# amidos2006/gym-pcgrl

Measured on AMD Instinct MI355X. Metric: env-steps/sec (whole node), binary-narrow 14x14 @ 65536 envs, higher is better.
Workload: dtype u8; 1 GPU; binary-narrow-v0 14x14, 65536 envs/GPU; envs_per_gpu=65536, width=14, height=14, max_changes=39, actions=uniform random, device-generated before the timed region, parallelism=env-axis shard x1, no collective on the step path

## Files before the change

gym_pcgrl_amd/_lib.py:

```python
import ctypes as C
import os
import subprocess

PKG = os.path.dirname(os.path.abspath(__file__))
ROOT = os.path.dirname(PKG)
CSRC = os.path.join(PKG, "csrc")
LIBDIR = os.path.join(PKG, "lib")
SO = os.path.join(LIBDIR, "libpcgrl_hip.so")
SOURCES = [os.path.join(CSRC, "pcgrl_abi.hip")]
HIPCC_FLAGS = ["--offload-arch=gfx950", "-O3", "-std=c++17", "-ffp-contract=off", "-fPIC", "-shared", "-mllvm", "-amdgpu-sched-strategy=max-ilp"]

PCGRL_OK, PCGRL_EINVAL, PCGRL_EHIP, PCGRL_ESTATE = 0, -1, -2, -3


class Config(C.Structure):
    _fields_ = [(n, C.c_int32) for n in (
        "prob", "rep", "num_envs", "width", "height", "prob_width", "prob_height", "max_changes", "max_iterations",
        "random_start", "random_tile", "warp", "random_probs", "auto_reset", "target_path",
        "max_enemies", "target_enemy_dist", "max_crates", "target_solution", "solver_power", "max_potions",
        "max_treasures", "max_diamonds", "min_spikes", "target_jumps", "min_empty", "min_enemies", "min_jumps")] + [
        ("target_col_enemies", C.c_double), ("tile_probs", C.c_double * 8), ("rewards", C.c_double * 12)]


class Layout(C.Structure):
    _fields_ = [(n, C.c_int32) for n in ("group", "mask_bytes", "nplanes", "nstats")] + [
        (n, C.c_size_t) for n in ("map", "old_map", "heatmap", "pos", "planes", "counters", "stats", "start_stats",
                                  "info", "reward", "done", "tile_p", "rng_rep", "rng_prob", "rng_cursor", "scratch")]


TUNING_FIELDS = ("no_fused", "fused_zelda", "step_epb", "no_inc", "inline_reset", "pair_min", "no_wide", "wide_waves", "wide_grid",
                 "wide_pairs", "wide_few", "sok_generic", "sok_hard_cap", "sok_spawn", "md_only_agent", "smb_lds_heap", "full_per_wave", "inc_per_wave", "wide_spin", "step_prio", "no_touch", "touch_tight", "step_pair", "async_split", "big_team", "obs_at_end")


class Tuning(C.Structure):
    _fields_ = [(n, C.c_int32) for n in TUNING_FIELDS]


TUNING_OVERRIDES = {}


def make_tuning(overrides=None):
    t = Tuning(*([-1] * len(TUNING_FIELDS)))
    for k, v in list(TUNING_OVERRIDES.items()) + list((overrides or {}).items()):
        if k not in TUNING_FIELDS:
            raise KeyError("unknown tuning switch %r (known: %s)" % (k, ", ".join(TUNING_FIELDS)))
        setattr(t, k, int(v))
    return t


BUFFER_NAMES = ("map", "old_map", "heatmap", "pos", "planes", "counters", "stats", "start_stats", "info", "reward",
                "done", "tile_p", "rng_rep", "rng_prob", "rng_cursor", "scratch")


class Buffers(C.Structure):
    _fields_ = [(n, C.c_void_p) for n in BUFFER_NAMES]


ROW_FIELDS = ("actions_out", "reward", "done", "start_in", "start_out", "ep_return", "ep_length", "took", "fresh")


class Row(C.Structure):
    _fields_ = [(n, C.c_void_p) for n in ROW_FIELDS] + [("actions_i64", C.c_int32)]


class RenderDesc(C.Structure):
    _fields_ = [("indices", C.c_void_p), ("count", C.c_int32), ("tiles", C.c_void_p), ("tile_size", C.c_int32),
                ("border_x", C.c_int32), ("border_y", C.c_int32), ("border_tile", C.c_int32), ("cursor", C.c_int32),
                ("grid_rows", C.c_int32), ("grid_cols", C.c_int32), ("out", C.c_void_p)]


ABI_VERSION = 15
EXPORTS = ("pcgrl_abi_version", "pcgrl_error_string", "pcgrl_last_hip_error", "pcgrl_query_layout", "pcgrl_create",
           "pcgrl_destroy", "pcgrl_bind", "pcgrl_configure", "pcgrl_seed", "pcgrl_set_tile_probs", "pcgrl_reset",
           "pcgrl_step", "pcgrl_set_maps", "pcgrl_observe", "pcgrl_action_map", "pcgrl_status", "pcgrl_profile",
           "pcgrl_profile_read", "pcgrl_bind_episode_stats", "pcgrl_seed_words", "pcgrl_rollout", "pcgrl_bind_observation", "pcgrl_selftest_heap",
           "pcgrl_tuning_defaults", "pcgrl_set_tuning", "pcgrl_clear_status", "pcgrl_step_flat",
           "pcgrl_async_bytes", "pcgrl_bind_async", "pcgrl_step_async", "pcgrl_async_flush", "pcgrl_step_multi", "pcgrl_selftest_step_pool", "pcgrl_step_threads", "pcgrl_selftest_range_reward",
           "pcgrl_bind_row", "pcgrl_render", "pcgrl_get_stats_bytes", "pcgrl_get_stats", "pcgrl_get_reward",
           "pcgrl_get_solution_bytes", "pcgrl_get_solution")
NPHASE = 6
PHASES = ("update", "stats", "reset_or_idle", "solver_or_reset", "reset2", "solver2")


def sources_newer_than_lib():
# ... 130 lines not shown
```

gym_pcgrl_amd/csrc/kernels_stats.h:

```cpp
#pragma once
template <class MaskT>
__device__ __forceinline__ MaskT row_valid(int lane, int W, int H) {
    MaskT full = (W >= (int)(8 * sizeof(MaskT))) ? ~(MaskT)0 : (((MaskT)1 << W) - 1);
    return lane < H ? full : (MaskT)0;
}

template <int PROB = -1>
__device__ __forceinline__ bool finalize_item(const PcgrlParams& P, const DevBufs& B, int e, const int32_t* s,
                                              int mode, int parity, int shard, bool push_reset = true, int rst_list = WL_RST,
                                              const int2* pre = nullptr, const double* reward_pre = nullptr) {
    const int prob = PROB >= 0 ? PROB : P.prob;
    int32_t* st = B.stats + (size_t)e * 8;
    int32_t* start = B.start_stats + (size_t)e * 8;
    if (mode == MODE_STEP) {
        int32_t old[PCGRL_MAX_STATS], sv[PCGRL_MAX_STATS];
        for (int k = 0; k < 8; k++) { old[k] = st[k]; sv[k] = start[k]; }
        const int2 c = pre ? *pre : reinterpret_cast<const int2*>(B.counters)[e];
        const double r = reward_pre ? *reward_pre : compute_reward(P, s, old, prob);
        const bool d = episode_over(P, s, sv, prob) || c.y >= P.max_changes || c.x >= P.max_iterations;
        B.reward[e] = r;
        B.done[e] = d ? 1 : 0;
        episode_account(B, e, r, d);
        int32_t* inf = B.info + (size_t)e * 10;
#pragma unroll
// ... 118 lines not shown
            MaskT t0, t1, t2;
            reset_rows_to_planes<MaskT>(P, reinterpret_cast<MaskT*>(B.planes) + (size_t)ek * NPL * G, gw == 2 * k + 1 ? g.lane : -1, rr.m0, rr.m1, rr.m2, t0, t1, t2);
            if (gw == 2 * k + 1) { b0 = t0; b1 = t1; b2 = t2; }
            __builtin_amdgcn_wave_barrier();
        }
        TL(9);
        const bool act = have && (role == 1 || !reset_only);
        int32_t sl[PCGRL_MAX_STATS] = {0, 0, 0, 0, 0, 0, 0, 0};
        MaskT champ_l = 0;
        bool ns = false;
        if (act) ns = compute_item_stats<PROB>(g, P, b0, b1, b2, rowmask, sl, champ_l, (B.step_tight & 2) != 0);
        TL(10);
        constexpr bool kLaneReward = PROB == PCGRL_PROB_ZELDA && G == 16;
        double rpre = 0.0;
        if (kLaneReward && SL && role == 0 && act) rpre = zelda_reward_lanes(&SL->zr, B.stats + (size_t)e * 8, sl, g.lane);
        if (g.lane == 0 && role == 0 && act) finalize_item<PROB>(P, B, e, sl, MODE_STEP, parity, shard, false, WL_RST, &pre, (kLaneReward && SL) ? &rpre : nullptr);
        __builtin_amdgcn_wave_barrier();
        if (role == 1 && have) {
            if (kInc && champ_base) champ_base[(size_t)e * G + g.lane] = champ_l;
            if (g.lane == 0) finish_or_park<PROB>(P, B, e, sl, ns, MODE_START, parity, shard);
        }
        if (FUSED && step_obs) {
#pragma unroll
            for (int k = 0; k < GPW / 2; k++) {
                if (k > 0 && !pair) break;
                if (!__builtin_amdgcn_readlane((int)have, 2 * k * G)) continue;
                const ObsPlanes<MaskT, NPL> src = {reinterpret_cast<const MaskT*>(B.planes), G};
                obs_write_env_lean(src, obs_view_from_lds(&SL->obs_v), B.pos, __builtin_amdgcn_readlane(e, 2 * k * G), lane64);
            }
        }
        return;
    }
    int32_t s[PCGRL_MAX_STATS] = {0, 0, 0, 0, 0, 0, 0, 0};
    bool need_solver = false;
    MaskT champ = 0;
    if (kInc && inc) {
        if (compute) {
            const MaskT cbit = (g.lane == wl_inc_row<G>(raw)) ? (MaskT)1 << wl_inc_col<G>(raw) : (MaskT)0;
            const MaskT champ_old = champ_base[(size_t)e * G + g.lane];
            const int4 old = *reinterpret_cast<const int4*>(B.stats + (size_t)e * 8);
            int regions, path, ub2;
            binary_incremental(g, (MaskT)(~b0 & rowmask), cbit, wl_inc_code<G>(raw) != 0, old.x, old.y, champ_old, old.w - 1, regions, path, champ, ub2);
            s[0] = regions; s[1] = path; s[2] = 1; s[3] = ub2 + 1;
        }
    } else if (kZinc && packed) {
        if (compute) {
            const MaskT cbit = (g.lane == wl_inc_row<G>(raw)) ? (MaskT)1 << wl_inc_col<G>(raw) : (MaskT)0;
            zelda_stats(g, P, b0, b1, b2, rowmask, s, (int)wl_inc_code<G>(raw), cbit, B.stats[(size_t)e * 8 + 4]);
        }
    } else {
        bool full = compute;
        if (kInc && G == 16) {
            const bool t = compute && tch;
            if (t) {
                const MaskT cbit = (g.lane == wl_inc_row<G>(raw)) ? (MaskT)1 << wl_inc_col<G>(raw) : (MaskT)0;
                const MaskT champ_old = champ_base[(size_t)e * G + g.lane];
                const int4 old = *reinterpret_cast<const int4*>(B.stats + (size_t)e * 8);
                int regions, path, ub2;
                if (binary_touch(g, (MaskT)(~b0 & rowmask), cbit, (wl_inc_code<G>(raw) & 1u) != 0, old.x, champ_old, old.w - 1, regions, path, champ, ub2)) {
                    s[0] = regions; s[1] = path; s[2] = 1; s[3] = ub2 + 1;
                    full = false;
                }
            }
        }
        if (full) need_solver = compute_item_stats<PROB>(g, P, b0, b1, b2, rowmask, s, champ, (B.step_tight & 1) != 0);
    }
    if (kInc && compute && champ_base) champ_base[(size_t)e * G + g.lane] = champ;
    TL(10);
    int want_reset = 0;
    constexpr bool kLaneReward = PROB == PCGRL_PROB_ZELDA && G == 16;
    double rpre = 0.0;
    const bool lane_reward = kLaneReward && SL != nullptr && mode == MODE_STEP;
    if (lane_reward && have && !reset_only) rpre = zelda_reward_lanes(&SL->zr, B.stats + (size_t)e * 8, s, g.lane);
    if (g.lane == 0 && have) {
        if (reset_only) want_reset = 1;
        else want_reset = finish_or_park<PROB>(P, B, e, s, need_solver, mode, parity, shard, !inline_reset, -1, lane_reward ? &rpre : nullptr) ? 1 : 0;
    }
    if (inline_reset) {
        const uint64_t want = __ballot(want_reset != 0);
        TL(11);
        if (want) {
            TL(12);
            if (SL) { while (__hip_atomic_load(&SL->refill_done[SL->par], __ATOMIC_ACQUIRE, __HIP_MEMORY_SCOPE_WORKGROUP) < SL->need) __builtin_amdgcn_s_sleep(2); }
            bool mine = false;
#pragma unroll
            for (int k = 0; k < GPW; k++) {
                if ((want >> (k * G)) & 1ull) {
                    const int ek = __builtin_amdgcn_readlane(e, k * G);
                    if (SL && lane64 == 0) { SL->dirty[ek - SL->e0] = 1; SL->late[ek - SL->e0] = 1; SL->n_late = 1; }
                    int pend = 0;
                    if (SL) {
                        if (lane64 == 0) {
                            pend = atomicExch(&SL->pend[ek - SL->e0], 0);
                            if (pend < 0) {
                                while (__hip_atomic_load(&SL->late_done[(ek - SL->e0) >> 6], __ATOMIC_ACQUIRE, __HIP_MEMORY_SCOPE_WORKGROUP) == 0) __builtin_amdgcn_s_sleep(2);
                                pend = 0;
                            }
                        }
                        pend = __builtin_amdgcn_readfirstlane(pend);
                    }
                    ResetRows rr;
                    wave_reset_env<PROB, !FUSED, FUSED>(P, B, ek, gen_map, mt, (uint8_t*)nullptr, lane64, 0, gw == k ? g.lane : -1, &rr, pend);
                    MaskT t0, t1, t2;
                    reset_rows_to_planes<MaskT>(P, reinterpret_cast<MaskT*>(B.planes) + (size_t)ek * NPL * G, gw == k ? g.lane : -1, rr.m0, rr.m1, rr.m2, t0, t1, t2);
                    if (gw == k) { b0 = t0; b1 = t1; b2 = t2; mine = true; }
                    __builtin_amdgcn_wave_barrier();
                }
            }
            if (mine) {
                int32_t st[PCGRL_MAX_STATS] = {0, 0, 0, 0, 0, 0, 0, 0};
                const bool ns = compute_item_stats<PROB>(g, P, b0, b1, b2, rowmask, st, champ, (B.step_tight & 2) != 0);
                if (kInc && champ_base) champ_base[(size_t)e * G + g.lane] = champ;
                if (g.lane == 0) finish_or_park<PROB>(P, B, e, st, ns, MODE_START, parity, shard);
            }
        }
// ... 316 lines not shown
```

gym_pcgrl_amd/csrc/pcgrl_abi.hip:

```cpp
#include <hip/hip_runtime.h>
#include <stdio.h>
#include <stdlib.h>
#include <string.h>

#include <vector>

#include "../../include/pcgrl_hip.h"

#ifdef PCGRL_PART
#define PCGRL_IN_PART(k) (PCGRL_PART == (k))
#else
#define PCGRL_IN_PART(k) 1
#endif
#define PCGRL_LOCAL __attribute__((visibility("hidden")))
#define PART_CORE 0
#define PART_STATS 1
#define PART_UPDATE 2
#define PART_STEP_BINARY 3
#define PART_STEP_ZELDA 4
#define PART_SEARCH 5
#define PART_SMB 6
#define PART_STEP_SOLVER 7

#include "lanegroup_dev.h"
// ... 222 lines not shown
        S.sok_env = b.take(align_up((size_t)c->num_envs * (SOK_RES_WORDS + SOK_CNT_WORDS + SOK_STOP_WORDS) * 4, 256));
        S.sok_sync = b.take(align_up(2 * (size_t)(SOK_SY_WORDS + SOK_HARD_CAP) * 4, 256));
        if (!big && !sok_in_lds(c)) {
            S.sok_heap = b.take(SOK_BLOCKS * sok_heap_bytes(c->solver_power));
            S.sok_table = b.take(SOK_BLOCKS * (size_t)sok_table_size(c->solver_power) * 4);
        }
    }
    S.champ = b.take(champ_bytes(c));
    const size_t n = (size_t)c->num_envs;
    S.fifo = b.take(c->rep == PCGRL_NARROW ? align_up(n * PCGRL_FIFO_N * 4, 256) : 0);
    S.fifo_tag = b.take(c->rep == PCGRL_NARROW ? align_up(n * 4, 256) : 0);
    S.wide_sync = b.take((c->prob == PCGRL_BINARY && c->height > 16 && !big_map(c)) ? align_up(n * 16, 256) : 0);
    S.total = b.off;
    return S;
}

PCGRL_LOCAL int search_device_setup(pcgrl_env* h);
PCGRL_LOCAL int smb_device_setup(pcgrl_env* h);
#if PCGRL_IN_PART(PART_CORE)
static int device_setup(pcgrl_env* h) {
    {
        uint32_t tab[PCGRL_MT_N];
        tab[0] = 19650218u;
        for (int i = 1; i < PCGRL_MT_N; i++) tab[i] = 1812433253u * (tab[i - 1] ^ (tab[i - 1] >> 30)) + (uint32_t)i;
        HIPCHK(hipMemcpyToSymbol(HIP_SYMBOL(g_mt_genrand), tab, sizeof(tab)));
    }
    if (h->cfg.prob == PCGRL_SMB) return smb_device_setup(h);
    if (solver_prob(h->cfg.prob) && !big_search(&h->cfg)) return search_device_setup(h);
    return PCGRL_OK;
}

static void resolve_tuning(pcgrl_env* h) {
    const pcgrl_tuning& T = h->tun;
    DevBufs& B = h->B;
    h->no_wide = tun_or(T.no_wide, 0) ? 1 : 0;
    h->wide_waves = tun_or(T.wide_waves, 8);
    h->wide_pairs = tun_or(T.wide_pairs, 1);
    h->wide_grid = tun_or(T.wide_grid, 2048);
    if (h->wide_grid < 1) h->wide_grid = 2048;
    h->fused_zelda = tun_or(T.fused_zelda, 1) ? 1 : 0;
    h->no_fused = tun_or(T.no_fused, 0) ? 1 : 0;
    h->obs_at_end = tun_or(T.obs_at_end, 0) ? 1 : 0;
    h->async_split = tun_or(T.async_split, h->cfg.prob == PCGRL_SOKOBAN ? 1 : 0) ? 1 : 0;
    const int n_ = h->cfg.num_envs;
    h->step_epb = T.step_epb > 0 ? T.step_epb : ((n_ >= 192 * 256 && n_ <= 256 * 256) ? 256 : (n_ >= 192 * 128 ? 128 : 64));
    if (h->step_epb != 128 && h->step_epb != 256) h->step_epb = 64;
    h->smb_heap = T.smb_lds_heap > 0 ? T.smb_lds_heap : SMB_LDS_HEAP;
    if (h->smb_heap < 256 || h->smb_heap > 4096) h->smb_heap = SMB_LDS_HEAP;
    const int f = tun_or(T.full_per_wave, 4), i = tun_or(T.inc_per_wave, 4);
    B.step_fpw = (f == 1 || f == 2) ? f : 4;
    B.step_prio = tun_or(T.step_prio, h->cfg.prob == PCGRL_BINARY ? (h->cfg.rep == PCGRL_NARROW ? (15 | (3 << 6)) : 15) : 0) & 0xFFF;
    B.step_ipw = (i == 1 || i == 2) ? i : 4;
    B.step_touch = tun_or(T.no_touch, 0) ? 0 : 1;
    B.step_pair = tun_or(T.step_pair, 6);
    B.step_tight = B.step_touch ? tun_or(T.touch_tight, 1) : 0;
    h->no_inc = tun_or(T.no_inc, 0) != 0;
    B.zelda_inc = (h->cfg.prob == PCGRL_ZELDA && h->cfg.rep <= PCGRL_REP_TURTLE && h->cfg.height <= 16 && h->cfg.width <= 32 &&
                   h->cfg.num_envs <= WL_INC_ENV_MASK && !h->no_inc) ? 1 : 0;
    B.pair_min = tun_or(T.pair_min, 2048);
    B.big_team = tun_or(T.big_team, 1) ? 1 : 0;
    h->big_team_waves = tun_or(T.big_team, 1) >= 2 ? (tun_or(T.big_team, 1) > BIG_TEAM_MAX_WAVES ? BIG_TEAM_MAX_WAVES : tun_or(T.big_team, 1)) : 4;
    B.wide_few = tun_or(T.wide_few, WL_WIDE_FEW_REGIONS);
    B.wide_spin = T.wide_spin > 0 ? T.wide_spin : WIDE_SPIN_LIMIT;
    B.inline_reset = (!solver_prob(h->cfg.prob) && tun_or(T.inline_reset, 1) != 0) ? 1 : 0;
    if (big_search(&h->cfg)) {
        B.sok_fast_maxc = -1; B.md_only_agent = -1; B.sok_hard_cap = 0; B.sok_spawn_iters = SOK_SPAWN_ITERS;
    } else if (solver_prob(h->cfg.prob)) {
        B.sok_fast_maxc = tun_or(T.sok_generic, 0) ? -1 : SOKF_MAXC;
        B.md_only_agent = T.md_only_agent;
        B.sok_hard_cap = tun_or(T.sok_hard_cap, SOK_HARD_CAP);
        B.sok_spawn_iters = T.sok_spawn > 0 ? T.sok_spawn : SOK_SPAWN_ITERS;
        if (B.sok_hard_cap > SOK_HARD_CAP) B.sok_hard_cap = SOK_HARD_CAP;
    }
}
static int bind_buffers(pcgrl_env* h, const pcgrl_buffers* b, hipStream_t st) {
    const pcgrl_config& c = h->cfg;
    DevBufs& B = h->B;
    B.map = (uint8_t*)b->map; B.old_map = (uint8_t*)b->old_map; B.heat = (uint16_t*)b->heatmap; B.pos = (uint8_t*)b->pos;
    B.heat_end = B.heat + (size_t)c.num_envs * c.width * c.height;
    B.heat32 = c.auto_reset ? 0 : 1;
    B.ep_return = nullptr; B.ep_length = nullptr; B.last_return = nullptr; B.last_length = nullptr;
    B.planes = b->planes; B.counters = (int32_t*)b->counters; B.stats = (int32_t*)b->stats;
    B.start_stats = (int32_t*)b->start_stats; B.info = (int32_t*)b->info; B.reward = (double*)b->reward;
    B.done = (uint8_t*)b->done; B.tile_p = (double*)b->tile_p; B.rng_rep = (uint32_t*)b->rng_rep;
    B.rng_prob = (uint32_t*)b->rng_prob; B.rng_cur = (int32_t*)b->rng_cursor;
    B.obs = ObsSpec{nullptr, 0, 0, 0, 0, 0, 0, 0};
    B.local = nullptr; B.flat = nullptr;
    const ScratchPlan S = scratch_plan(&c);
    uint8_t* s = (uint8_t*)b->scratch;
    B.wl_cnt = at<int32_t>(s, S.wl_cnt); B.status = at<int32_t>(s, S.status);
    for (int k = 0; k < WL_NLIST; k++) { B.wl_cap[k] = wl_capacity(c.num_envs, k); B.wl_items[k] = at<int32_t>(s, S.wl_items[k]); }
    HIPCHK(hipMemsetAsync(B.wl_cnt, 0, S.wl_cnt.bytes + S.status.bytes, st));
    B.champ = h->no_inc ? nullptr : at<uint8_t>(s, S.champ);
    if (B.champ) HIPCHK(hipMemsetAsync(B.champ, c.prob == PCGRL_SMB ? 0xFF : 0, S.champ.bytes, st));
    B.fifo = at<uint32_t>(s, S.fifo); B.fifo_tag = at<int32_t>(s, S.fifo_tag);
    if (B.fifo_tag) HIPCHK(hipMemsetAsync(B.fifo_tag, 0xFF, S.fifo_tag.bytes, st));
    B.wide_sync = at<int32_t>(s, S.wide_sync); B.wide_epoch = 0;
    if (B.wide_sync) HIPCHK(hipMemsetAsync(B.wide_sync, 0, S.wide_sync.bytes, st));
    const bool big = big_search(&c);
    B.big_arena = big ? at<uint8_t>(s, S.arena) : nullptr;
    B.sok_pool = big ? nullptr : at<SokNode>(s, S.arena);
    B.sok_heap = at<uint32_t>(s, S.sok_heap); B.sok_table = at<uint32_t>(s, S.sok_table);
    if (solver_prob(c.prob)) {
        const int power = h->alloc_solver_power = c.solver_power;
        h->big_dims = S.big;
        B.sok_res = at<int32_t>(s, S.sok_env);
// ... 1243 lines not shown
```

gym_pcgrl_amd/csrc/pcgrl_algos.h:

```cpp
#pragma once
#include "pcgrl_common.h"

#if defined(__HIPCC__) && defined(__HIP_DEVICE_COMPILE__)
#define PCGRL_NO_IFCVT() asm volatile("" ::: "memory")
#else
#define PCGRL_NO_IFCVT() do {} while (0)
#endif
#ifndef PCGRL_TRACE
#define PCGRL_TRACE(g, site)
#endif

struct PcgrlParams {
    int32_t prob, rep, num_envs, width, height, ntiles, nplanes, group, mask_bytes;
    int32_t max_changes, max_iterations;
    int32_t random_start, random_tile, warp, random_probs, auto_reset;
    int32_t target_path, max_enemies, target_enemy_dist, max_crates, target_solution, solver_power;
    int32_t prob_width, prob_height;
    int32_t max_potions, max_treasures;
    int32_t max_diamonds, min_spikes, target_jumps;
    int32_t min_empty, min_enemies, min_jumps;
    int32_t big, big_search;
    double target_col_enemies;
    double rewards[PCGRL_MAX_REWARDS];
    double cdf[PCGRL_MAX_TILES];
// ... 374 lines not shown
template <class B>
PCGRL_D void regions_and_longest_path(B& g, typename B::mask_t pass, int& regions, int& path) {
    typename B::mask_t champ;
    regions_and_longest_path(g, pass, regions, path, champ);
}

template <class B>
PCGRL_D void binary_incremental(B& g, typename B::mask_t pass_new, typename B::mask_t cbit, bool added, int regions_old, int path_old,
                                typename B::mask_t champ_old, int ub2_old, int& regions, int& path, typename B::mask_t& champ, int& ub2) {
    typedef typename B::mask_t M;
    const M base = pass_new & ~cbit;
    M rest = pcg_neighbours(g, cbit) & base;
    path = path_old;
    champ = champ_old;
    constexpr bool kTrack = B::kGroup == 16;
    const bool track = kTrack && ub2_old >= 0;
    int k = 0, ub = track ? ub2_old : 0;
    M uni = cbit;
    if (g.any(rest)) {
        const PcgFillCtx<B> ctx = pcg_fill_ctx(g, base);
        while (g.any(rest)) {
            const M comp = pcg_component(g, g.first_bit(rest), ctx);
            rest = rest & ~comp;
            ++k;
            if (added) uni = uni | comp;
            else {
                int bd = g.popcount_sum(comp) - 1, e = 0;
                const int thr = track ? ub : path;
                if (bd > thr) e = pcg_double_sweep(g, comp, thr, bd);
                if (e > path) { if (kTrack) ub = path > ub ? path : ub; path = e; champ = comp; }
                else if (kTrack) ub = bd > ub ? bd : ub;
            }
        }
    }
    if (added) {
        regions = regions_old + 1 - k;
        int bd = g.popcount_sum(uni) - 1, e = 0;
        const int thr = track ? ub : path;
        if (bd > thr) e = pcg_double_sweep(g, uni, thr, bd);
        if (e > path) { if (kTrack) ub = path > ub ? path : ub; path = e; champ = uni; }
        else if (kTrack) ub = bd > ub ? bd : ub;
    } else {
        regions = regions_old + k - 1;
    }
    ub2 = track ? ub : -1;
}
template <class B>
PCGRL_D void binary_incremental(B& g, typename B::mask_t pass_new, typename B::mask_t cbit, bool added, int regions_old, int path_old,
                                typename B::mask_t champ_old, int& regions, int& path, typename B::mask_t& champ) {
    int ub2;
    binary_incremental(g, pass_new, cbit, added, regions_old, path_old, champ_old, -1, regions, path, champ, ub2);
}

template <class B>
PCGRL_D bool binary_touch(B& g, typename B::mask_t pass_new, typename B::mask_t cbit, bool added, int regions_old,
                          typename B::mask_t champ_old, int ub2_old, int& regions, int& path, typename B::mask_t& champ, int& ub2) {
    typedef typename B::mask_t M;
    const M base = pass_new & ~cbit;
    const M dom = added ? (base & ~champ_old) : (champ_old & ~cbit);
    M rest = pcg_neighbours(g, cbit) & dom;
    int k = 0, size1 = 0, size2 = 0, size3 = 0;
    M uni = cbit ^ cbit, big1 = uni, big2 = uni;
    if (g.any(rest)) {
        const PcgFillCtx<B> ctx = pcg_fill_ctx(g, dom);
        while (g.any(rest)) {
            const M comp = pcg_component(g, g.first_bit(rest), ctx);
            rest = rest & ~comp;
            ++k;
            uni = uni | comp;
            const int size = g.popcount_sum(comp);
            if (size > size1) { size3 = size2; size2 = size1; big2 = big1; size1 = size; big1 = comp; }
            else if (size > size2) { size3 = size2; size2 = size; big2 = comp; }
            else if (size > size3) size3 = size;
        }
    }
    const M target = added ? (champ_old | cbit | uni) : big1;
    int e = pcg_double_sweep(g, target, added ? ub2_old - 1 : -1);
    bool ok = true;
    int ub = ub2_old;
    champ = target;
    if (added) {
        regions = regions_old - k;
    } else {
        regions = regions_old + k - 1;
        ok = k > 0;
        if (size2 > 0) {
            int bd = size2 - 1, e2 = 0;
            const int thr = e < ub ? e : ub;
            if (bd > thr) e2 = pcg_double_sweep(g, big2, thr, bd);
            if (e2 > e) { ub = e > ub ? e : ub; e = e2; champ = big2; }
            else ub = bd > ub ? bd : ub;
        }
        if (size3 > 0) {
            if (size3 - 1 > e) ok = false;
            else ub = size3 - 1 > ub ? size3 - 1 : ub;
        }
    }
    path = e;
    ub2 = ub;
    return ok && e >= ub2_old;
}

template <class B>
PCGRL_D typename B::mask_t rlp_choose_seed(B& g, typename B::mask_t rest, int row_lo, int row_hi) {
    const typename B::mask_t mine = g.rows_between(rest, row_lo, row_hi);
    return g.first_bit(g.any(mine) ? mine : rest);
}
#if defined(PCGRL_TIMELINE) && defined(__HIPCC__)
__device__ __forceinline__ void tl_mark(int tag);
#define PCGRL_TLA(tag) tl_mark(tag)
#else
#define PCGRL_TLA(tag) do {} while (0)
#endif
#if defined(__HIPCC__) && defined(__HIP_DEVICE_COMPILE__) && !defined(PCGRL_EXP_NO_SWEEP_PRIO)
#define PCGRL_SWEEP_PRIO(p) __builtin_amdgcn_s_setprio(p)
#else
#define PCGRL_SWEEP_PRIO(p) do {} while (0)
#endif
template <class B, class Shared>
PCGRL_D void rlp_process_seed(B& g, typename B::mask_t seed, const PcgFillCtx<B>& ctx, Shared& sh, int& regions, int& my_best,
                              typename B::mask_t& my_champ) {
    typedef typename B::mask_t M;
    const M comp = pcg_component(g, seed, ctx);
    PCGRL_TLA(30);
    if (!sh.retire(g, comp)) return;
    ++regions;
    const int best = sh.best();
    if (g.popcount_sum(comp) - 1 > best) {
        PCGRL_TLA(31);
        PCGRL_SWEEP_PRIO(3);
        const int e = pcg_double_sweep(g, comp, best);
        PCGRL_SWEEP_PRIO(0);
        if (e > my_best) { my_best = e; my_champ = comp; }
        sh.raise(e);
        PCGRL_TLA(32);
    }
}
template <class B, class Shared>
PCGRL_D void rlp_process_seed(B& g, typename B::mask_t seed, const PcgFillCtx<B>& ctx, Shared& sh, int& regions) {
    int my_best = 0;
    typename B::mask_t my_champ = seed ^ seed;
    rlp_process_seed(g, seed, ctx, sh, regions, my_best, my_champ);
}
template <class B>
PCGRL_D typename B::mask_t rlp_prepare(B& g, typename B::mask_t pass, int& tiny_regions, int& tiny_path) {
    tiny_regions = 0; tiny_path = 0;
    return pass & ~pcg_tiny_components(g, pass, tiny_regions, tiny_path);
}

template <class M>
struct ZeldaMasks {
    M empty, solid, player, key, door, enemy;
};
// ... 137 lines not shown
```

gym_pcgrl_amd/csrc/worklist.h:

```cpp
#pragma once
#define PCGRL_BLOCK 256
#define PCGRL_STATUS_TOO_MANY_CRATES 1
#define PCGRL_STATUS_BAD_ACTION 2
#define PCGRL_STATUS_BAD_TILE 4
enum { MODE_STEP = 0, MODE_START = 1, MODE_SETMAP = 2 };

#define WL_NSHARD 64
#define WL_WIDE_FEW_REGIONS 32
#define WL_CSTRIDE 16
enum { WL_CHG = 0, WL_RST = 1, WL_SOL = 2, WL_SOL2 = 3, WL_RST2 = 4, WL_SOL3 = 5, WL_INC = 6, WL_NLIST = 7 };
#ifndef SMB_LONG_POPS
#define SMB_LONG_POPS 2000
#endif
#define WL_INC_ENV_MASK 0x1FFFFF
#define WL_INC64_ENV_MASK 0x7FFFF
__device__ __forceinline__ int wl_inc_pack(int group, int e, int row, int col, unsigned code) {
    return group == 16 ? (int)((unsigned)e | ((unsigned)(row * 32 + col) << 21) | (code << 30))
                       : (int)((unsigned)e | ((unsigned)(row * 64 + col) << 19) | ((code & 1u) << 31));
}
#define WL_INCBIG_ENV_MASK 0x7FFF
__device__ __forceinline__ int wl_incbig_pack(int e, int x, int y, bool added) { return (int)((unsigned)e | ((unsigned)x << 15) | ((unsigned)y << 23) | (added ? 0x80000000u : 0u)); }
template <int G> __device__ __forceinline__ int wl_inc_env(int raw) { return raw & (G == 16 ? WL_INC_ENV_MASK : WL_INC64_ENV_MASK); }
template <int G> __device__ __forceinline__ int wl_inc_row(int raw) { return G == 16 ? ((raw >> 26) & 15) : ((raw >> 25) & 63); }
template <int G> __device__ __forceinline__ int wl_inc_col(int raw) { return G == 16 ? ((raw >> 21) & 31) : ((raw >> 19) & 63); }
// ... 19 lines not shown
        const int i = s_tl_idx[wv];
        if (i < TL_SLOTS) { g_tl_buf[((size_t)blockIdx.x * (blockDim.x >> 6) + wv) * TL_SLOTS + i] = ((unsigned long long)wall_clock64() << 8) | (unsigned)tag; s_tl_idx[wv] = i + 1; }
    }
}
#define TL_INIT() do { if ((threadIdx.x & 63) == 0) s_tl_idx[threadIdx.x >> 6] = 0; } while (0)
#define TL(tag) tl_mark(tag)
#else
#define TL_INIT() do {} while (0)
#define TL(tag) do {} while (0)
#endif

struct LocalLists;
struct ObsSpec { uint8_t* out; int32_t oh, ow, depth, centered, pad;
                 int32_t fused,
                         delta; };
struct RowBind { int64_t* actions_out; double* reward; uint8_t* done; const uint8_t* start_in; uint8_t* start_out;
                 double* ep_return; int32_t* ep_length; uint8_t* took; uint8_t* fresh; };
struct DevBufs {
    uint8_t* map; uint8_t* old_map; uint16_t* heat; uint8_t* pos; void* planes;
    void* champ;
    int32_t* wide_sync;
    int32_t wide_spin;
    int32_t wide_few;
    int32_t wide_epoch;
    const uint16_t* heat_end;
    double* ep_return; int32_t* ep_length; double* last_return; int32_t* last_length;
    int32_t* counters; int32_t* stats; int32_t* start_stats; int32_t* info;
    double* reward; uint8_t* done; double* tile_p;
    uint32_t* rng_rep; uint32_t* rng_prob; int32_t* rng_cur;
    int32_t* wl_cnt;
    int32_t* wl_items[WL_NLIST];
    int32_t wl_cap[WL_NLIST];
    SokNode* sok_pool; uint32_t* sok_heap; uint32_t* sok_table; int32_t* status;
    int32_t* sok_res;
    int32_t* sok_cnt; int32_t* sok_stop;
    struct LocalLists* local;
    int32_t md_only_agent;
    int32_t* sok_sync;
    int32_t sok_pool_stride, sok_heap_stride, sok_table_size, sok_use_lds;
    int32_t sok_spawn_iters;
    int32_t sok_hard_cap;
    int32_t sok_fast_maxc;
    int32_t inline_reset;
    int32_t pair_min;
    int32_t zelda_inc;
    uint32_t* fifo; int32_t* fifo_tag;
    ObsSpec obs;
    int32_t step_fpw, step_ipw;
    int32_t step_prio;
    int32_t step_tight;
    const int32_t* flat;
    int32_t step_pair;
    int32_t big_team;
    int32_t step_touch;
    uint8_t* big_arena;
    uint8_t* pending; unsigned long long* async_stats;
    const uint8_t* async_slots; size_t async_slot_bytes; int32_t async_nslots; int32_t* async_run; int32_t* async_run_n;
    int32_t heat32;
    RowBind row; int32_t act_i64;
};
#define PCGRL_FIFO_N 8

struct ZeldaRewardTab { double w[8]; int lo[8]; int hi[8]; };
struct ObsView {
    uint8_t* out;
    int oh, ow, depth, centered, pad, W, H;
};
struct StepLocal {
    int e0;
    int par, need;
    int refill_done[2];
    int pend[256];
    int late_done[4];
    uint8_t dirty[256];
    uint8_t obs_skip[256];
    uint8_t late[256];
    int n_late;
    ObsView obs_v;
    ZeldaRewardTab zr;
};

__device__ __forceinline__ void async_list_runnable(const DevBufs& B, int gi) {
    if (gi < B.async_nslots && __hip_atomic_load(reinterpret_cast<const int32_t*>(B.async_slots + (size_t)gi * B.async_slot_bytes), __ATOMIC_RELAXED, __HIP_MEMORY_SCOPE_AGENT) == 1)
        B.async_run[atomicAdd(B.async_run_n, 1)] = gi;
}
__device__ __forceinline__ int32_t* wl_counters(const DevBufs& B, int parity, int list) {
    return B.wl_cnt + (size_t)(parity * WL_NLIST + list) * WL_NSHARD * WL_CSTRIDE;
}
#define WL_LOCAL_CAP 512
struct LocalLists { int n[WL_NLIST]; int e0; uint16_t items[WL_NLIST][WL_LOCAL_CAP]; };
__device__ __forceinline__ void wl_push(const DevBufs& B, int parity, int list, int shard, int value) {
    if (B.local) {
        const int i = atomicAdd(&B.local->n[list], 1);
        B.local->items[list][i] = (uint16_t)(value - B.local->e0);
        return;
    }
    const int i = atomicAdd(wl_counters(B, parity, list) + shard * WL_CSTRIDE, 1);
    B.wl_items[list][(size_t)shard * B.wl_cap[list] + i] = value;
}
__device__ __forceinline__ int wl_load_prefix(const DevBufs& B, int parity, int list, int* s_pref) {
    if (threadIdx.x < WL_NSHARD) {
        int v = wl_counters(B, parity, list)[threadIdx.x * WL_CSTRIDE];
        for (int o = 1; o < WL_NSHARD; o <<= 1) {
            const int t = __shfl_up(v, o, 64);
            if ((int)threadIdx.x >= o) v += t;
        }
// ... 163 lines not shown
```

include/pcgrl_hip.h:

```cpp
#ifndef PCGRL_HIP_H
#define PCGRL_HIP_H
#include <stddef.h>
#include <stdint.h>

#ifdef __cplusplus
extern "C" {
#endif

#define PCGRL_ABI_VERSION 15
#define PCGRL_OK 0
#define PCGRL_EINVAL (-1)
#define PCGRL_EHIP (-2)
#define PCGRL_ESTATE (-3)

enum { PCGRL_BINARY = 0, PCGRL_ZELDA = 1, PCGRL_SOKOBAN = 2, PCGRL_MDUNGEON = 3, PCGRL_DDAVE = 4, PCGRL_SMB = 5 };
enum { PCGRL_NARROW = 0, PCGRL_WIDE = 1, PCGRL_TURTLE = 2, PCGRL_NARROW_CAST = 3, PCGRL_NARROW_MULTI = 4, PCGRL_TURTLE_CAST = 5 };

typedef struct pcgrl_config {
    int32_t prob, rep;
    int32_t num_envs;
    int32_t width, height;
    int32_t prob_width, prob_height;
    int32_t max_changes, max_iterations;
    int32_t random_start, random_tile, warp, random_probs;
// ... 16 lines not shown
    int32_t nstats;
    size_t map;
    size_t old_map;
    size_t heatmap;
    size_t pos;
    size_t planes;
    size_t counters;
    size_t stats;
    size_t start_stats;
    size_t info;
    size_t reward;
    size_t done;
    size_t tile_p;
    size_t rng_rep;
    size_t rng_prob;
    size_t rng_cursor;
    size_t scratch;
} pcgrl_layout;

typedef struct pcgrl_buffers {
    void *map, *old_map, *heatmap, *pos, *planes, *counters, *stats, *start_stats, *info, *reward,
         *done, *tile_p, *rng_rep, *rng_prob, *rng_cursor, *scratch;
} pcgrl_buffers;

typedef struct pcgrl_env pcgrl_env;

typedef struct pcgrl_tuning {
    int32_t no_fused;
    int32_t fused_zelda;
    int32_t step_epb;
    int32_t no_inc;
    int32_t inline_reset;
    int32_t pair_min;
    int32_t no_wide;
    int32_t wide_waves;
    int32_t wide_grid;
    int32_t wide_pairs;
    int32_t wide_few;
    int32_t sok_generic;
    int32_t sok_hard_cap;
    int32_t sok_spawn;
    int32_t md_only_agent;
    int32_t smb_lds_heap;
    int32_t full_per_wave;
    int32_t inc_per_wave;
    int32_t wide_spin;
    int32_t step_prio;
    int32_t no_touch;
    int32_t touch_tight;
    int32_t step_pair;
    int32_t async_split;
    int32_t big_team;
    int32_t obs_at_end;
} pcgrl_tuning;

int pcgrl_abi_version(void);
const char* pcgrl_error_string(int code);
int pcgrl_last_hip_error(void);

int pcgrl_query_layout(const pcgrl_config* cfg, pcgrl_layout* out);
int pcgrl_create(const pcgrl_config* cfg, pcgrl_env** out);
int pcgrl_destroy(pcgrl_env* env);
void pcgrl_tuning_defaults(pcgrl_tuning* t);
int pcgrl_set_tuning(pcgrl_env* env, const pcgrl_tuning* t);
int pcgrl_bind(pcgrl_env* env, const pcgrl_buffers* bufs, void* stream);
int pcgrl_configure(pcgrl_env* env, const pcgrl_config* cfg);
int pcgrl_seed(pcgrl_env* env, const uint32_t* keys, int32_t first, int32_t count, void* stream);
int pcgrl_seed_words(pcgrl_env* env, const uint32_t* words, int32_t first, int32_t count, void* stream);
int pcgrl_set_tile_probs(pcgrl_env* env, void* stream);
int pcgrl_reset(pcgrl_env* env, void* stream);
int pcgrl_step(pcgrl_env* env, const int32_t* actions, void* stream);
int pcgrl_step_multi(pcgrl_env* const* envs, const int32_t* const* actions, void* const* streams, int32_t count);
int32_t pcgrl_step_threads(int32_t n);
int pcgrl_rollout(pcgrl_env* env, const int32_t* actions, int32_t steps, double* reward_out, uint8_t* done_out,
                  int32_t* info_out, void* stream);
int pcgrl_set_maps(pcgrl_env* env, const uint8_t* maps, void* stream);
int pcgrl_observe(pcgrl_env* env, uint8_t* out, int32_t out_h, int32_t out_w, int32_t centered, int32_t pad_value,
                  int32_t onehot, void* stream);
int pcgrl_bind_observation(pcgrl_env* env, uint8_t* out, int32_t out_h, int32_t out_w, int32_t centered,
                           int32_t pad_value, int32_t onehot, int32_t incremental);
typedef struct pcgrl_row {
    int64_t* actions_out;
    double*  reward;
    uint8_t* done;
    const uint8_t* start_in;
    uint8_t* start_out;
    double*  ep_return;
    int32_t* ep_length;
    uint8_t* took;
    uint8_t* fresh;
    int32_t  actions_i64;
} pcgrl_row;
int pcgrl_bind_row(pcgrl_env* env, const pcgrl_row* row);
typedef struct pcgrl_render_desc {
    const int32_t* indices;
    int32_t count;
    const uint8_t* tiles;
    int32_t tile_size;
    int32_t border_x, border_y, border_tile, cursor;
    int32_t grid_rows, grid_cols;
    uint8_t* out;
} pcgrl_render_desc;
int pcgrl_render(pcgrl_env* env, const pcgrl_render_desc* d, void* stream);
size_t pcgrl_get_stats_bytes(const pcgrl_config* cfg, int32_t count);
int    pcgrl_get_stats(pcgrl_env* env, const uint8_t* maps, int32_t count, int32_t* rows_out,
                       void* work, size_t work_bytes, void* stream);
// ... 30 lines not shown
```

Baseline: 2.309 billion env-steps/s.

## Resume longest-path search from touch-pass memo instead of full recompute

When the incremental touch update of the binary path/region stats cannot conclude, the step now resumes the region and longest-path computation from a memo of components and double-sweep results already found, instead of falling back to the full compute_item_stats pass. The resume skips re-sweeping known components and prunes remaining components by size bounds. This adds a new switch (on by default, only for the fused 32-bit mask path) and more register state carried through the touch routine, which could raise register pressure or introduce correctness risk in the bound logic.

```diff
diff --git a/gym_pcgrl_amd/_lib.py b/gym_pcgrl_amd/_lib.py
--- a/gym_pcgrl_amd/_lib.py
+++ b/gym_pcgrl_amd/_lib.py
@@ -29,7 +29,7 @@
 
 
 TUNING_FIELDS = ("no_fused", "fused_zelda", "step_epb", "no_inc", "inline_reset", "pair_min", "no_wide", "wide_waves", "wide_grid",
-                 "wide_pairs", "wide_few", "sok_generic", "sok_hard_cap", "sok_spawn", "md_only_agent", "smb_lds_heap", "full_per_wave", "inc_per_wave", "wide_spin", "step_prio", "no_touch", "touch_tight", "step_pair", "async_split", "big_team", "obs_at_end")
+                 "wide_pairs", "wide_few", "sok_generic", "sok_hard_cap", "sok_spawn", "md_only_agent", "smb_lds_heap", "full_per_wave", "inc_per_wave", "wide_spin", "step_prio", "no_touch", "touch_tight", "step_pair", "async_split", "big_team", "obs_at_end", "touch_resume")
 
 
 class Tuning(C.Structure):
diff --git a/gym_pcgrl_amd/csrc/kernels_stats.h b/gym_pcgrl_amd/csrc/kernels_stats.h
--- a/gym_pcgrl_amd/csrc/kernels_stats.h
+++ b/gym_pcgrl_amd/csrc/kernels_stats.h
@@ -194,15 +194,31 @@
         bool full = compute;
         if (kInc && G == 16) {
             const bool t = compute && tch;
+            TouchMemo<MaskT> memo = touch_memo_empty(g, b0);
             if (t) {
                 const MaskT cbit = (g.lane == wl_inc_row<G>(raw)) ? (MaskT)1 << wl_inc_col<G>(raw) : (MaskT)0;
                 const MaskT champ_old = champ_base[(size_t)e * G + g.lane];
                 const int4 old = *reinterpret_cast<const int4*>(B.stats + (size_t)e * 8);
                 int regions, path, ub2;
-                if (binary_touch(g, (MaskT)(~b0 & rowmask), cbit, (wl_inc_code<G>(raw) & 1u) != 0, old.x, champ_old, old.w - 1, regions, path, champ, ub2)) {
+                if (binary_touch(g, (MaskT)(~b0 & rowmask), cbit, (wl_inc_code<G>(raw) & 1u) != 0, old.x, champ_old, old.w - 1, regions, path, champ, ub2, memo)) {
                     s[0] = regions; s[1] = path; s[2] = 1; s[3] = ub2 + 1;
                     full = false;
                 }
+            }
+#ifdef PCGRL_TIMELINE
+            {
+                const uint64_t gu = __ballot(t && full && g.lane == 0), pl = __ballot(compute && !tch && g.lane == 0);
+                TL(32 + __popcll(gu) + 8 * __popcll(pl));
+            }
+#endif
+            constexpr bool kResume = FUSED && sizeof(MaskT) == 4;
+            if (kResume && B.touch_resume) {
+                if (full) {
+                    int regions, path, ub2;
+                    rlp_resume(g, (MaskT)(~b0 & rowmask), memo, regions, path, champ, ub2, (B.step_tight & 1) != 0);
+                    s[0] = regions; s[1] = path; s[2] = g.any(champ) ? 1 : 0; s[3] = ub2 + 1;
+                }
+                full = false;
             }
         }
         if (full) need_solver = compute_item_stats<PROB>(g, P, b0, b1, b2, rowmask, s, champ, (B.step_tight & 1) != 0);
diff --git a/gym_pcgrl_amd/csrc/pcgrl_abi.hip b/gym_pcgrl_amd/csrc/pcgrl_abi.hip
--- a/gym_pcgrl_amd/csrc/pcgrl_abi.hip
+++ b/gym_pcgrl_amd/csrc/pcgrl_abi.hip
@@ -298,6 +298,7 @@
     B.step_prio = tun_or(T.step_prio, h->cfg.prob == PCGRL_BINARY ? (h->cfg.rep == PCGRL_NARROW ? (15 | (3 << 6)) : 15) : 0) & 0xFFF;
     B.step_ipw = (i == 1 || i == 2) ? i : 4;
     B.step_touch = tun_or(T.no_touch, 0) ? 0 : 1;
+    B.touch_resume = tun_or(T.touch_resume, 1) ? 1 : 0;
     B.step_pair = tun_or(T.step_pair, 6);
     B.step_tight = B.step_touch ? tun_or(T.touch_tight, 1) : 0;
     h->no_inc = tun_or(T.no_inc, 0) != 0;
diff --git a/gym_pcgrl_amd/csrc/pcgrl_algos.h b/gym_pcgrl_amd/csrc/pcgrl_algos.h
--- a/gym_pcgrl_amd/csrc/pcgrl_algos.h
+++ b/gym_pcgrl_amd/csrc/pcgrl_algos.h
@@ -450,9 +450,23 @@
     binary_incremental(g, pass_new, cbit, added, regions_old, path_old, champ_old, -1, regions, path, champ, ub2);
 }
 
+template <class M>
+struct TouchMemo {
+    M comp1, comp2;
+    int val1, bd1, val2, bd2, bd3, regions, k;
+    bool valid;
+};
+template <class B>
+PCGRL_D TouchMemo<typename B::mask_t> touch_memo_empty(B& g, typename B::mask_t any_mask) {
+    TouchMemo<typename B::mask_t> m;
+    m.comp1 = any_mask ^ any_mask; m.comp2 = m.comp1;
+    m.val1 = 0; m.bd1 = -1; m.val2 = 0; m.bd2 = -1; m.bd3 = -1; m.regions = 0; m.k = 0; m.valid = false;
+    return m;
+}
 template <class B>
 PCGRL_D bool binary_touch(B& g, typename B::mask_t pass_new, typename B::mask_t cbit, bool added, int regions_old,
-                          typename B::mask_t champ_old, int ub2_old, int& regions, int& path, typename B::mask_t& champ, int& ub2) {
+                          typename B::mask_t champ_old, int ub2_old, int& regions, int& path, typename B::mask_t& champ, int& ub2,
+                          TouchMemo<typename B::mask_t>& memo) {
     typedef typename B::mask_t M;
     const M base = pass_new & ~cbit;
     const M dom = added ? (base & ~champ_old) : (champ_old & ~cbit);
@@ -473,10 +487,13 @@
         }
     }
     const M target = added ? (champ_old | cbit | uni) : big1;
-    int e = pcg_double_sweep(g, target, added ? ub2_old - 1 : -1);
+    int bd1 = 0;
+    int e = pcg_double_sweep(g, target, added ? ub2_old - 1 : -1, bd1);
     bool ok = true;
     int ub = ub2_old;
     champ = target;
+    memo.comp1 = target; memo.val1 = e; memo.bd1 = bd1;
+    memo.comp2 = uni ^ uni; memo.val2 = 0; memo.bd2 = -1; memo.bd3 = -1; memo.k = k; memo.valid = true;
     if (added) {
         regions = regions_old - k;
     } else {
@@ -486,17 +503,98 @@
             int bd = size2 - 1, e2 = 0;
             const int thr = e < ub ? e : ub;
             if (bd > thr) e2 = pcg_double_sweep(g, big2, thr, bd);
+            memo.comp2 = big2; memo.val2 = e2; memo.bd2 = bd;
             if (e2 > e) { ub = e > ub ? e : ub; e = e2; champ = big2; }
             else ub = bd > ub ? bd : ub;
         }
         if (size3 > 0) {
+            memo.bd3 = size3 - 1;
             if (size3 - 1 > e) ok = false;
             else ub = size3 - 1 > ub ? size3 - 1 : ub;
         }
-    }
+        if (k == 0) { memo.comp1 = uni ^ uni; memo.val1 = 0; memo.bd1 = -1; }
+    }
+    memo.regions = regions;
     path = e;
     ub2 = ub;
     return ok && e >= ub2_old;
+}
+template <class B>
+PCGRL_D bool binary_touch(B& g, typename B::mask_t pass_new, typename B::mask_t cbit, bool added, int regions_old,
+                          typename B::mask_t champ_old, int ub2_old, int& regions, int& path, typename B::mask_t& champ, int& ub2) {
+    TouchMemo<typename B::mask_t> memo;
+    return binary_touch(g, pass_new, cbit, added, regions_old, champ_old, ub2_old, regions, path, champ, ub2, memo);
+}
+
+template <class B>
+PCGRL_D void rlp_resume(B& g, typename B::mask_t pass, const TouchMemo<typename B::mask_t>& memo, int& regions, int& path,
+                        typename B::mask_t& champ, int& ub2, bool tight = true) {
+    typedef typename B::mask_t M;
+    typedef typename B::ivec_t I;
+    regions = 0;
+    path = 0;
+    champ = pass ^ pass;
+    const M nontiny = pass & ~pcg_tiny_components(g, pass, regions, path);
+    const bool known = memo.valid;
+    int ub = path;
+    if (known && memo.val1 > 0) {
+        if (memo.val1 > path) { path = memo.val1; champ = memo.comp1; }
+    }
+    if (known && memo.val2 > 0) {
+        if (memo.val2 > path) { ub = path > ub ? path : ub; path = memo.val2; champ = memo.comp2; }
+        else ub = memo.val2 > ub ? memo.val2 : ub;
+    } else if (known && memo.bd2 > ub) ub = memo.bd2;
+    const bool pend1 = known && memo.val1 <= 0 && g.any(memo.comp1);
+    M rest = nontiny & ~memo.comp1 & ~memo.comp2;
+    M big1 = pend1 ? memo.comp1 : (pass ^ pass), big2 = pass ^ pass;
+    int size1 = 0, size2 = 0, size3 = 0;
+    const int count = known ? 0 : 1;
+    if (known) regions = memo.regions;
+    if (pend1) { size1 = g.popcount_sum(memo.comp1); size1 = memo.bd1 + 1 < size1 ? memo.bd1 + 1 : size1; }
+    if (g.any(rest)) {
+        const PcgFillCtx<B> ctx = pcg_fill_ctx(g, pass);
+        while (g.any(rest)) {
+            if (count == 0) {
+                const int n = g.popcount_sum(rest);
+                if (n - 1 <= path) { ub = n - 1 > ub ? n - 1 : ub; break; }
+            }
+            const I cnt = g.popc_lanes(rest);
+            const M comp = pcg_component(g, g.first_bit(g.keep_where_eq(cnt, g.imax(cnt), rest)), ctx);
+            rest = rest & ~comp;
+            regions += count;
+            const int size = g.popcount_sum(comp);
+            if (size > size1) { size3 = size2; size2 = size1; big2 = big1; size1 = size; big1 = comp; }
+            else if (size > size2) { size3 = size2; size2 = size; big2 = comp; }
+            else if (size > size3) size3 = size;
+        }
+    }
+    int b1 = size1 - 1, b2 = size2 - 1;
+    if (b1 > path) {
+        const int e = pcg_double_sweep(g, big1, path, b1);
+        if (e > path) { ub = path > ub ? path : ub; path = e; champ = big1; b1 = -1; }
+    }
+    {
+        int rest_b = size3 - 1 > ub ? size3 - 1 : ub;
+        rest_b = b1 > rest_b ? b1 : rest_b;
+        if (b2 > path) {
+            const int e = pcg_double_sweep(g, big2, path, b2);
+            if (e > path) { ub = path > ub ? path : ub; path = e; champ = big2; b2 = -1; }
+        } else if (tight && b2 > rest_b) pcg_double_sweep(g, big2, rest_b, b2);
+    }
+    if (size3 - 1 > path) {
+        rest = nontiny & ~champ & ~big1 & ~big2;
+        const PcgFillCtx<B> ctx = pcg_fill_ctx(g, pass);
+        while (g.any(rest)) {
+            const M comp = pcg_component(g, g.first_bit(rest), ctx);
+            rest = rest & ~comp;
+            if (g.popcount_sum(comp) - 1 > path) {
+                const int e = pcg_double_sweep(g, comp, path);
+                if (e > path) { ub = path > ub ? path : ub; path = e; champ = comp; }
+            }
+        }
+    }
+    ub = b1 > ub ? b1 : ub; ub = b2 > ub ? b2 : ub; ub = size3 - 1 > ub ? size3 - 1 : ub;
+    ub2 = ub > path ? path : ub;
 }
 
 template <class B>
diff --git a/gym_pcgrl_amd/csrc/worklist.h b/gym_pcgrl_amd/csrc/worklist.h
--- a/gym_pcgrl_amd/csrc/worklist.h
+++ b/gym_pcgrl_amd/csrc/worklist.h
@@ -95,6 +95,7 @@
     const int32_t* flat;
     int32_t step_pair;
     int32_t big_team;
+    int32_t touch_resume;
     int32_t step_touch;
     uint8_t* big_arena;
     uint8_t* pending; unsigned long long* async_stats;
diff --git a/include/pcgrl_hip.h b/include/pcgrl_hip.h
--- a/include/pcgrl_hip.h
+++ b/include/pcgrl_hip.h
@@ -92,6 +92,7 @@
     int32_t async_split;
     int32_t big_team;
     int32_t obs_at_end;
+    int32_t touch_resume;
 } pcgrl_tuning;
 
 int pcgrl_abi_version(void);
```

Measured after the change: 2.405 billion env-steps/s, median of 6. +4.2%, better.
